# soedinglab/plass

Hardware: AMD Instinct MI355X
Metric: read-overlaps/s per assembly iteration (higher is better)
Workload: dtype u8/u64 (integer hash, byte compare; f32 ratios)

## Files before the change

### plass_amd/csrc/kmermatch.hip

```cpp
#include "common.hpp"
#include "device_utils.hpp"
#include "host_util.hpp"
#include "linepart.hpp"
#include "ref_rules.hpp"
#include "xxh64_u64.hpp"
#include <algorithm>
#include <memory>
#include <type_traits>
#include <cstdlib>
#include <climits>
#include <cstring>

namespace plasship {

#include "kmermatch_extract.hpp"
#include "kmermatch_group.hpp"
#include "kmermatch_repsort.hpp"
}
using namespace plasship;

namespace {

struct Timer {
    plasship_ctx *ctx; int slot;
// ... 72 lines not shown
    g.PL1 = pieceLinesFor(g.totalLines, g.nb1, numCU, 8);
    g.nP1 = (g.totalLines + g.PL1 - 1) / g.PL1;
    g.cap1 = std::max<uint64_t>(g.nP1 * ((uint64_t) g.PL1 + g.nb1), 1);
    if (g.nb2) {
        g.PL2 = 0xFFFFFFFFu; g.maxP2 = g.nb1; g.cap2 = g.cap1 + (uint64_t) g.nb1 * g.nb2;
    }
    return g;
}
static uint64_t repLevel1Cap(uint64_t nRec, uint64_t nSeg, uint32_t PL, uint32_t nb) {
    const uint64_t lines = (nRec + RPL - 1) / RPL + nSeg;
    return lines + (lines / PL + nSeg + 1) * (uint64_t) nb;
}

__global__ void arenaStartKernel(const uint32_t *__restrict__ lineBeg, uint32_t bpb, uint32_t gGrid, uint32_t nBuckets, uint64_t *__restrict__ arenaStart) {
    for (uint32_t j = blockIdx.x * blockDim.x + threadIdx.x; j < gGrid; j += gridDim.x * blockDim.x)
        arenaStart[j] = (uint64_t) lineBeg[std::min(j * bpb, nBuckets - 1)] * RPL;
}
__global__ void bigNeedKernel(const uint32_t *__restrict__ lineCnt, const uint32_t *__restrict__ unique, uint32_t nBuckets, uint64_t *__restrict__ need, uint32_t wordsPerEntry) {
    for (uint32_t b = blockIdx.x * blockDim.x + threadIdx.x; b < nBuckets; b += gridDim.x * blockDim.x) {
        const uint64_t c = (uint64_t) lineCnt[b] * RPL;
        uint64_t v = 0;
        if (unique[b] == AGG_NEEDS_SCRATCH) { uint64_t P = 1; while (P < c) P <<= 1; v = wordsPerEntry * P; }
        need[b] = v;
    }
}
__global__ void sumU32Kernel(const uint32_t *__restrict__ v, uint32_t n, unsigned long long *__restrict__ out) {
    unsigned long long s = 0;
    for (uint32_t i = blockIdx.x * blockDim.x + threadIdx.x; i < n; i += gridDim.x * blockDim.x) s += v[i];
    s = waveReduceSumU64(s);
    if (laneId() == 0 && s) atomicAdd(out, s);
}

template <class K> static int setDynLds(K k, size_t bytes) {
    PH_CHECK(hipFuncSetAttribute(reinterpret_cast<const void *>(k), hipFuncAttributeMaxDynamicSharedMemorySize, (int) bytes));
    return PLASSHIP_OK;
}
template <bool NUCL, bool LONG, int MODE, bool LIST, bool EXTRAS>
static int launchLinePart(plasship_ctx *ctx, const LinePartArgs &a, uint64_t nPiecesBound) {
    const size_t lds = linePartLdsBytes(a.nb, sizeof(Rec<LONG>), EXTRAS);
    const bool big = lds > 72 * 1024;
    const unsigned grid = (unsigned) std::max<uint64_t>(1, std::min<uint64_t>(nPiecesBound, (uint64_t) ctx->numCU * (big ? 1u : 2u)));
    if (big) {
        constexpr bool HASH = MODE == KEY_HASH;
        auto k = linePartKernel<NUCL, LONG, MODE, LIST, EXTRAS, 1024, (HASH && !LIST) ? 2 : 4, true, HASH, HASH>;
        const int rc = setDynLds(k, lds); if (rc) return rc;
        hipLaunchKernelGGL(k, dim3(grid), dim3(1024), lds, ctx->stream, a);
    } else {
        auto k = linePartKernel<NUCL, LONG, MODE, LIST, EXTRAS, 512, 4, true>;
        const int rc = setDynLds(k, lds); if (rc) return rc;
        hipLaunchKernelGGL(k, dim3(grid), dim3(512), lds, ctx->stream, a);
    }
    return PLASSHIP_OK;
}

static bool lineListDebugOn() { return getenv("PLASSHIP_DEBUG_LINELIST") != nullptr; }

static int buildLineLists(plasship_ctx *ctx, const char *who, const uint32_t *dTags, uint64_t capLines, uint32_t nb, uint32_t *dCount, uint32_t *dStart, uint32_t *dCursor, uint32_t *dList) {
    hipStream_t st = ctx->stream;
    PH_CHECK(hipMemsetAsync(dCount, 0, (size_t) nb * 4, st));
    const unsigned g = (unsigned) std::max<uint64_t>(1, std::min<uint64_t>((capLines + 4095) / 4096, (uint64_t) ctx->numCU * 8));
    const size_t lds = listRunsLdsBytes(LR_CHUNK, false);
    const unsigned gs = (unsigned) std::max<uint64_t>(1, std::min<uint64_t>((capLines + LR_CHUNK - 1) / LR_CHUNK, (uint64_t) ctx->numCU));
    auto k = tagScatterRunsKernel<LR_BLOCK, LR_CHUNK>;
    const int rc = setDynLds(k, lds); if (rc) return rc;
    hipLaunchKernelGGL(tagHistKernel, dim3(g), dim3(256), 0, st, dTags, capLines, nb, dCount);
    hipLaunchKernelGGL(tagScanKernel, dim3(1), dim3(1024), 0, st, (const uint32_t *) dCount, nb, dStart, dCursor);
    hipLaunchKernelGGL(k, dim3(gs), dim3(LR_BLOCK), lds, st, dTags, capLines, nb, dCursor, dList);
    if (lineListDebugOn()) {
        std::vector<uint32_t> s((size_t) nb + 1);
        PH_COPY_SYNC(st, s.data(), dStart, s.size() * 4, hipMemcpyDeviceToHost);
        uint32_t mx = 0; for (uint32_t b = 0; b < nb; b++) mx = std::max(mx, s[b + 1] - s[b]);
        fprintf(stderr, "lineList %s level 1 buckets %u lines %llu listed %u chunk %d chunks %llu regions 0 maxBucket %u\n", who, nb, (unsigned long long) capLines, s[nb], LR_CHUNK,
                (unsigned long long) ((capLines + LR_CHUNK - 1) / LR_CHUNK), mx);
    }
    return PLASSHIP_OK;
}
static int buildRegionLists(plasship_ctx *ctx, const char *who, const uint32_t *dTags, const uint32_t *dNPieces, const uint64_t *dRegBeg, const uint64_t *dRegEnd, uint32_t nRegions, uint32_t nb2, uint32_t *dList, uint32_t *dFineBeg, uint32_t *dFineCnt) {
    hipStream_t st = ctx->stream;
    const size_t lds = listRunsLdsBytes(LR2_CHUNK, true);
    auto k = tagSortRegionRunsKernel<LR2_BLOCK, LR2_CHUNK>;
    const int rc = setDynLds(k, lds); if (rc) return rc;
    hipLaunchKernelGGL(k, dim3(std::max<uint32_t>(1, std::min<uint32_t>(nRegions, (uint32_t) ctx->numCU))), dim3(LR2_BLOCK), lds, st, dTags, dRegBeg, dRegEnd, nRegions, nb2, dList, dFineBeg, dFineCnt);
    if (lineListDebugOn()) {
        std::vector<uint64_t> rb(nRegions), re(nRegions); std::vector<uint32_t> fc((size_t) nRegions * nb2);
        PH_COPY_SYNC(st, rb.data(), dRegBeg, rb.size() * 8, hipMemcpyDeviceToHost); PH_COPY_SYNC(st, re.data(), dRegEnd, re.size() * 8, hipMemcpyDeviceToHost);
        PH_COPY_SYNC(st, fc.data(), dFineCnt, fc.size() * 4, hipMemcpyDeviceToHost);
        uint32_t nPieces = 0; PH_COPY_SYNC(st, &nPieces, dNPieces, 4, hipMemcpyDeviceToHost);
        uint64_t lines = 0, listed = 0, chunks = 0, maxRegion = 0; uint32_t mx = 0, emptyRegions = 0;
        for (uint32_t g = 0; g < nRegions; g++) {
            const uint64_t len = re[g] - rb[g]; lines += len; chunks += (len + LR2_CHUNK - 1) / LR2_CHUNK;
            uint64_t in = 0; for (uint32_t f = 0; f < nb2; f++) { const uint32_t c = fc[(size_t) g * nb2 + f]; in += c; mx = std::max(mx, c); }
            listed += in; maxRegion = std::max(maxRegion, in); emptyRegions += in == 0;
        }
        fprintf(stderr, "lineList %s level 2 buckets %u lines %llu listed %llu chunk %d chunks %llu regions %u maxBucket %u emptyRegions %u maxRegion %llu pieces %u\n", who, nb2, (unsigned long long) lines,
                (unsigned long long) listed, LR2_CHUNK, (unsigned long long) chunks, nRegions, mx, emptyRegions, (unsigned long long) maxRegion, nPieces);
    }
    return PLASSHIP_OK;
}

static bool shardOwnerFiltered(int W) { const int m = tuneInt("SHARD_EXTRACT", 0); return m == 2 || (m != 1 && W <= 4); }

constexpr int KM_RETRY_EARLY_OVERFLOW_CHECK = -1000;
struct LinesOut { void *triples = nullptr; uint64_t nTriples = 0, Nk = 0, Nm = 0; std::vector<int64_t> stalePos; uint32_t staleT = 0; float msSort1 = 0, msGroup = 0, msSort2 = 0, msPart = 0; int nPart = 1;
                  uint64_t exchangedRecordBytes = 0, exchangedTripleBytes = 0; };

constexpr uint64_t HALO_SLACK = 1u << 16;
// ... 738 lines not shown
        bool fast = k == KF;
        uint64_t pwH = 1; for (int i = 0; i < HF; i++) pwH *= sa.base;
        if (pwH * 2 >= (1ull << 32)) fast = false;
        sa.topLo = (uint32_t) (pwH / sa.base); sa.topHi = (uint32_t) ea.powers[KF - HF - 1]; sa.baseH = (uint32_t) pwH;
        const dim3 shortGrid(std::min<uint32_t>((nMine + 63) / 64, (uint32_t) ctx->numCU * (nMine > 20000000u ? 288u : 18u)));
        const bool allWork = (int64_t) db->maxEntryLen - 2 - k + 1 <= (int64_t) par->kmers_per_seq - 1;
        const size_t padLds = (size_t) (allWork ? 16 : 8) << 10;
        const bool staged = !LONG && allWork;
        if (fast && sa.base < (1u << 8) && sa.topLo < (1u << 24) && sa.topHi < (1u << 24) && staged) {
            if constexpr (!LONG) hipLaunchKernelGGL((extractShortFastKernel<LONG, KF, true, true>), shortGrid, dim3(64), 0, st, sa);
        }
        else if (fast && sa.base < (1u << 8) && sa.topLo < (1u << 24) && sa.topHi < (1u << 24)) hipLaunchKernelGGL((extractShortFastKernel<LONG, KF, true>), shortGrid, dim3(64), padLds, st, sa);
        else if (fast) hipLaunchKernelGGL((extractShortFastKernel<LONG, KF, false>), shortGrid, dim3(64), 0, st, sa);
        else hipLaunchKernelGGL((extractShortKernel<LONG>), shortGrid, dim3(64), 0, st, sa);
        ea.waveList = dWaveList.as<uint32_t>(); ea.waveCount = dWaveCount.as<uint32_t>();
        if (cacheReuse) {
            CachedArgs ca; memset(&ca, 0, sizeof(ca));
            ca.s = ea.s; ca.slotOff = ea.slotOff; ca.arr = ea.arr; ca.map = ea.map; ca.lines = kc.lines.as<unsigned char>();
            ca.list = dCachedList.as<uint32_t>(); ca.count = dCachedCount.as<uint32_t>(); ca.k = k; ca.xCode = ea.xCode;
            ca.base = (uint32_t) ea.powers[1]; ca.base7 = (uint32_t) ea.powers[7]; ca.slotBias = slotBias; ca.seed = ea.seed; ca.kstats = dKStats.as<unsigned long long>();
            hipLaunchKernelGGL(extractCachedKernel, dim3(std::min<uint32_t>(nMine, (uint32_t) ctx->numCU * 32u)), dim3(64), 0, st, ca);
        }
    }
    else if (nMine) {
        hipLaunchKernelGGL(classifyWindowsKernel, dim3(std::min<uint32_t>((nMine + 2047) / 2048, (uint32_t) ctx->numCU * 8)), dim3(256), 0, st, (const uint32_t *) db->d_len.as<uint32_t>(), sLo, sHi, (uint32_t) k,
                           TIER0_WINDOWS, 64u * 16u, dWaveList.as<uint32_t>(), dWaveCount.as<uint32_t>(), dLongList.as<uint32_t>(), dLongCount.as<uint32_t>(), dOvIds.as<uint32_t>(), dOvCnt.as<uint32_t>(),
                           posReuse ? (const uint32_t *) db->d_origin.as<uint32_t>() : (const uint32_t *) nullptr, dCachedList.as<uint32_t>(), dCachedCount.as<uint32_t>());
        ea.waveList = dWaveList.as<uint32_t>(); ea.waveCount = dWaveCount.as<uint32_t>();
        if constexpr (NUCL) {
            if (posReuse) {
                CachedPosArgs<LONG> ca; memset(&ca, 0, sizeof(ca));
                ca.s = ea.s; ca.slotOff = ea.slotOff; ca.arr = ea.arr; ca.map = ea.map; ca.posOld = pc.pos.p; ca.slotOffOld = pc.slotOff.as<uint64_t>();
                ca.idHashOld = pc.idHash.as<unsigned long long>(); ca.origin = db->d_origin.as<uint32_t>(); ca.posNew = dPosNew.p; ca.idHashNew = dIdHashNew.as<unsigned long long>();
                ca.list = dCachedList.as<uint32_t>(); ca.count = dCachedCount.as<uint32_t>(); ca.k = k; ca.seed = ea.seed; ca.kstats = dKStats.as<unsigned long long>();
                hipLaunchKernelGGL((extractCachedPosKernel<LONG>), dim3(std::min<uint32_t>(nMine, (uint32_t) ctx->numCU * 32u)), dim3(64), 0, st, ca);
            }
        }
    }
    PH_CHECK(hipEventRecord(ctx->ev[3], st));
    PH_CHECK(hipEventRecord(ctx->ev[4], st));
    const int waveBlocksPerCU = nMine > 5000000u ? 192 : 32;
    DevBuf dOv2Ids, dOv2Cnt;
    DevBuf *lastIds = &dOvIds, *lastCnt = &dOvCnt;
    if (nMine) {
        if (dOv2Ids.alloc(((size_t) N + 1) * 4) != hipSuccess || dOv2Cnt.alloc(4) != hipSuccess) { setError("kmermatch: out of device memory"); return PLASSHIP_ERR_DEVICE; }
        PH_CHECK(hipMemsetAsync(dOv2Cnt.p, 0, 4, st));
        const uint32_t wide = std::min<uint32_t>(nMine, (uint32_t) ctx->numCU * (uint32_t) waveBlocksPerCU);
        ExtractArgs e0 = ea;
        DevBuf dRowLists, dRowCounts, dRowFall, dRowFallCnt;
        const bool rowTier = !NUCL && !LONG && fastIndex && k <= 14 && par->kmers_per_seq >= 1 && par->kmers_per_seq <= (int) KMC_POS + 1 &&
                             par->kmers_per_seq_scale == 0.0f && (tuneInt("ROWTIER", nMine > 4000000u ? 1 : 2) & 1) == 1;
        if (rowTier) {
            const uint32_t rs = N + 1;
            if (dRowLists.alloc((size_t) 4 * rs * 4) != hipSuccess || dRowCounts.alloc(16) != hipSuccess || dRowFall.alloc((size_t) rs * 4) != hipSuccess || dRowFallCnt.alloc(4) != hipSuccess) {
                setError("kmermatch: out of device memory"); return PLASSHIP_ERR_DEVICE;
            }
            PH_CHECK(hipMemsetAsync(dRowCounts.p, 0, 16, st));
            PH_CHECK(hipMemsetAsync(dRowFallCnt.p, 0, 4, st));
            hipLaunchKernelGGL(binWaveListKernel, dim3(std::min<uint32_t>((nMine + 2047) / 2048, (uint32_t) ctx->numCU * 8)), dim3(256), 0, st, (const uint32_t *) dWaveList.as<uint32_t>(), (const uint32_t *) dWaveCount.as<uint32_t>(),
                               (const uint32_t *) db->d_len.as<uint32_t>(), (uint32_t) k, 96u, 128u, 192u, dRowLists.as<uint32_t>(), rs, dRowCounts.as<uint32_t>());
            RowArgs ra; memset(&ra, 0, sizeof(ra));
            ra.s = ea.s; ra.slotOff = ea.slotOff; ra.arr = ea.arr; ra.map = ea.map; ra.fallList = dRowFall.as<uint32_t>(); ra.fallCount = dRowFallCnt.as<uint32_t>();
            ra.k = k; ra.xCode = ea.xCode; ra.kps = ea.kps; ra.ignoreMulti = ea.ignoreMulti; ra.seed = ea.seed; ra.base = (uint32_t) ea.powers[1]; ra.base7 = (uint32_t) ea.powers[7];
            ra.slotBias = slotBias; ra.kstats = dKStats.as<unsigned long long>();
            const dim3 rowGrid(std::min<uint32_t>((nMine + 3) / 4, (uint32_t) ctx->numCU * 32u));
            for (int b = 0; b < 4; b++) {
                ra.list = dRowLists.as<uint32_t>() + (size_t) b * rs; ra.count = dRowCounts.as<uint32_t>() + b;
                if (b == 0) hipLaunchKernelGGL((extractRowKernel<6>), rowGrid, dim3(64), 0, st, ra);
                else if (b == 1) hipLaunchKernelGGL((extractRowKernel<8>), rowGrid, dim3(64), 0, st, ra);
                else if (b == 2) hipLaunchKernelGGL((extractRowKernel<12>), rowGrid, dim3(64), 0, st, ra);
                else hipLaunchKernelGGL((extractRowKernel<16>), rowGrid, dim3(64), 0, st, ra);
            }
            e0.waveList = dRowFall.as<uint32_t>(); e0.waveCount = dRowFallCnt.as<uint32_t>();
        }
        hipLaunchKernelGGL((extractKernel<NUCL, LONG, CAP, false, 4, 256>), dim3(wide), dim3(64), 0, st, e0);
        ExtractArgs e1 = ea; e1.waveList = dLongList.as<uint32_t>(); e1.waveCount = dLongCount.as<uint32_t>();
        hipLaunchKernelGGL((extractKernel<NUCL, LONG, CAP, false, 16, 992>), dim3(wide), dim3(64), 0, st, e1);
        ExtractArgs e2 = ea; e2.waveList = dOvIds.as<uint32_t>(); e2.waveCount = dOvCnt.as<uint32_t>();
        e2.overflowIds = dOv2Ids.as<uint32_t>(); e2.overflowCount = dOv2Cnt.as<uint32_t>();
        constexpr int CAP48 = NUCL ? 512 : 128;
        if constexpr (NUCL) hipLaunchKernelGGL((extractKernel<NUCL, LONG, CAP48, false, 48, 992, 2>), dim3(std::min<uint32_t>(nMine, (uint32_t) ctx->numCU * 8u)), dim3(64), 0, st, e2);
        else hipLaunchKernelGGL((extractKernel<NUCL, LONG, CAP2, false, 48, 992>), dim3(std::min<uint32_t>(nMine, (uint32_t) ctx->numCU * 16u)), dim3(64), 0, st, e2);
        PH_CHECK(hipMemsetAsync(dOvCnt.p, 0, 4, st));
        ExtractArgs e3 = ea; e3.waveList = dOv2Ids.as<uint32_t>(); e3.waveCount = dOv2Cnt.as<uint32_t>();
        e3.overflowIds = dOvIds.as<uint32_t>(); e3.overflowCount = dOvCnt.as<uint32_t>();
        hipLaunchKernelGGL((extractKernel<NUCL, LONG, CAP2, false, 0, 8160>), dim3(std::min<uint32_t>(nMine, (uint32_t) ctx->numCU * (NUCL ? 2u : 5u))), dim3(64), 0, st, e3);
    }
    DevBuf &dLastIds = *lastIds, &dLastCnt = *lastCnt;
    PH_CHECK(hipEventRecord(ctx->ev[5], st));
    uint32_t nOv = 0;
    const bool overflowPossible = overflowCheckEarly || cm != nullptr || NUCL || db->maxEntryLen > 8160u || par->kmers_per_seq > 120 || par->kmers_per_seq_scale != 0.0f;
    if (nMine && overflowPossible) {
        PH_CHECK(hipMemcpyAsync(&nOv, dLastCnt.p, 4, hipMemcpyDeviceToHost, st));
        PH_CHECK(plasship::streamSync(st));
    } else if (nMine) hipLaunchKernelGGL((fillOverflowSlotsKernel<LONG>), dim3(64), dim3(64), 0, st, (const uint32_t *) dLastIds.as<uint32_t>(), (const uint32_t *) dLastCnt.as<uint32_t>(),
                                         (const uint64_t *) dSlotOff.as<uint64_t>(), slotBias, dA.p);
    PH_CHECK(hipGetLastError());
    if (nOv) {
        std::vector<uint32_t> ids(nOv), lens(nOv);
        DevBuf dLens, dSOff, dSCap, dScratch;
        if (dLens.alloc((size_t) nOv * 4) != hipSuccess) { setError("kmermatch: out of device memory"); return PLASSHIP_ERR_DEVICE; }
        hipLaunchKernelGGL(gatherU32Kernel, dim3(gridFor(nOv, 256, 1024)), dim3(256), 0, st, db->d_len.as<uint32_t>(), dLastIds.as<uint32_t>(), nOv, dLens.as<uint32_t>());
        PH_CHECK(hipMemcpyAsync(lens.data(), dLens.p, (size_t) nOv * 4, hipMemcpyDeviceToHost, st));
        PH_CHECK(plasship::streamSync(st));
        std::vector<uint64_t> soff(nOv); std::vector<uint32_t> scap(nOv); uint64_t tot = 0;
        for (uint32_t i = 0; i < nOv; i++) { uint32_t c = 64; while (c < lens[i] + 1) c <<= 1; scap[i] = c; soff[i] = tot; tot += c; }
        if (dSOff.alloc((size_t) nOv * 8) != hipSuccess || dSCap.alloc((size_t) nOv * 4) != hipSuccess || dScratch.alloc(tot * sizeof(Cand)) != hipSuccess) {
            setError("kmermatch: out of device memory for the long-sequence scratch"); return PLASSHIP_ERR_DEVICE;
        }
        PH_CHECK(hipMemcpyAsync(dSOff.p, soff.data(), (size_t) nOv * 8, hipMemcpyHostToDevice, st));
        PH_CHECK(hipMemcpyAsync(dSCap.p, scap.data(), (size_t) nOv * 4, hipMemcpyHostToDevice, st));
        ExtractArgs fa = ea; fa.idList = dLastIds.as<uint32_t>(); fa.nIds = nOv; fa.scratch = dScratch.as<Cand>(); fa.scratchOff = dSOff.as<uint64_t>(); fa.scratchCap = dSCap.as<uint32_t>();
        hipLaunchKernelGGL((extractKernel<NUCL, LONG, 1, true>), dim3(std::min<uint32_t>(nOv, (uint32_t) ctx->numCU * 8)), dim3(64), 0, st, fa);
        PH_CHECK(plasship::streamSync(st));
        PH_CHECK(hipGetLastError());
    }
    PH_TRACE(st, "kmermatch: extraction");
    traceBadIds<LONG>(ctx, "kmermatch: extracted slots", dA.p, total, N);

    {
        int keyBitsL = 0;
        if (NUCL) keyBitsL = 2 * k; else { long double v = 1; for (int i = 0; i < k; i++) v *= (long double) (alph - 1); while (keyBitsL < 63 && (long double) (1ULL << keyBitsL) < v) keyBitsL++; }
        LinesOut lo;
        int rcL = kmermatchLines<NUCL, LONG>(ctx, db, par, geo, total, dA, dB, dSlotOff, dKStats, ea, keyBitsL, lo, (nMine && !overflowPossible) ? dLastCnt.as<uint32_t>() : nullptr, filtered);
        if (rcL) return rcL;
        std::unique_ptr<plasship_cands> holderL; uint64_t NcL = 0; float msReduceL = 0;
        rcL = reduceToCandidates<NUCL, LONG>(ctx, db, lo.triples, lo.nTriples, lo.stalePos, lo.staleT, holderL, NcL, msReduceL, true);
        if (rcL) return rcL;
        {
            auto ms = [&](int a, int b) { float v = 0; (void) hipEventElapsedTime(&v, ctx->ev[a], ctx->ev[b]); return v; };
// ... 51 lines not shown
```

### plass_amd/csrc/kmermatch_extract.hpp

```cpp
#pragma once

__device__ __forceinline__ uint64_t revComplementDev(uint64_t kmer, int k) {
    uint64_t x = kmer ^ 0xAAAAAAAAAAAAAAAAULL;
    x = ((x >> 2) & 0x3333333333333333ULL) | ((x & 0x3333333333333333ULL) << 2);
    x = ((x >> 4) & 0x0F0F0F0F0F0F0F0FULL) | ((x & 0x0F0F0F0F0F0F0F0FULL) << 4);
    x = __builtin_bswap64(x);
    return x >> (64 - 2 * k);
}

__global__ void boundsKernel(const uint32_t *__restrict__ len, uint32_t n, int k, int kps, float scale, uint32_t *__restrict__ bound) {
    for (uint32_t i = blockIdx.x * blockDim.x + threadIdx.x; i < n; i += gridDim.x * blockDim.x) {
        const int L = (int) len[i];
        const int adj = max(1, L - k + 2);
        bound[i] = (uint32_t) min(adj, (int) ((float) (size_t) kps + (scale * (float) L)));
    }
}

struct Cand { uint64_t kmer; uint32_t pos; uint32_t score; };
constexpr uint32_t KMC_LINE = 128, KMC_POS = 59, KMC_FLAGS = 63, KMC_CLEAN = 1;

#define FALLBACK_NOSTATS(a) ((a).kstats == nullptr)
struct ExtractArgs {
    SeqView s;
    const uint64_t *slotOff;
// ... 915 lines not shown
        m.idh = *reinterpret_cast<const unsigned long long *>(ln);
        return m;
    };
    Meta nxt; nxt.id = 0; nxt.L = 0; nxt.pos = 0xFFFFu; nxt.off = 0; nxt.slot = 0; nxt.slot1 = 0; nxt.idh = 0;
    uint32_t id2 = 0;
    if (blockIdx.x < nWork) nxt = loadMeta(a.list[blockIdx.x]);
    if (blockIdx.x + gridDim.x < nWork) id2 = a.list[blockIdx.x + gridDim.x];
    for (uint32_t w = blockIdx.x; w < nWork; w += gridDim.x) {
        const Meta cur = nxt;
        if (w + gridDim.x < nWork) nxt = loadMeta(id2);
        if (w + 2 * gridDim.x < nWork) id2 = a.list[w + 2 * gridDim.x];
        const char *base = a.s.data + cur.off;
        const uint32_t bound = (uint32_t) (cur.slot1 - cur.slot);
        const bool have = cur.pos != 0xFFFFu;
        const uint32_t n = (uint32_t) __popcll(__ballot(have));
        if (have) {
            uint64_t r0, r1; __builtin_memcpy(&r0, base + cur.pos, 8); __builtin_memcpy(&r1, base + cur.pos + 8, 8);
            uint64_t w0 = 0, w1 = 0;
#pragma unroll
            for (int b = 0; b < 8; b++) { w0 |= (uint64_t) sMap[(r0 >> (8 * b)) & 0xFF] << (8 * b); w1 |= (uint64_t) sMap[(r1 >> (8 * b)) & 0xFF] << (8 * b); }
            uint64_t kmer; (void) kmerIndexCore(w0, w1, a.k, (unsigned) a.xCode, a.base, a.base7, kmer);
            R r; r.kmer = kmer; r.id = cur.id; r.len = (uint16_t) cur.L; r.pos = (int16_t) cur.pos;
            arr[cur.slot + 1 + (uint32_t) lane] = r;
        }
        if (lane == 63) { R r; r.kmer = xxh64U64(cur.idh, a.seed); r.id = cur.id; r.len = (uint16_t) cur.L; r.pos = 0; arr[cur.slot] = r; }
        for (uint32_t i = 1 + n + (uint32_t) lane; i < bound; i += 64) { R r; memset(&r, 0xFF, sizeof(R)); arr[cur.slot + i] = r; }
        stRes += cur.L; stRec += 1 + n;
    }
    if (lane == 0 && a.kstats) { atomicAdd(&a.kstats[2], stRes); atomicAdd(&a.kstats[3], stRec); }
}

struct RowArgs {
    SeqView s; const uint64_t *slotOff; void *arr; const unsigned char *map;
    const uint32_t *list, *count;
    uint32_t *fallList, *fallCount;
    int k, xCode, kps, ignoreMulti; uint64_t seed; uint32_t base, base7; uint64_t slotBias;
    unsigned long long *kstats;
};
constexpr uint64_t rowPowU64(uint64_t b, unsigned e) { uint64_t r = 1; while (e) { if (e & 1u) r *= b; b *= b; e >>= 1; } return r; }
constexpr uint64_t rowInv31() { uint64_t x = 31; for (int i = 0; i < 6; i++) x *= 2ull - 31ull * x; return x; }
static_assert(rowInv31() * 31ull == 1ull, "inverse of 31 modulo 2^64");
__device__ __forceinline__ uint32_t rowExclusiveScan16(uint32_t v) {
    uint32_t x = v;
    x += (uint32_t) __builtin_amdgcn_update_dpp(0, (int) x, 0x111, 0xF, 0xF, true);
    x += (uint32_t) __builtin_amdgcn_update_dpp(0, (int) x, 0x112, 0xF, 0xF, true);
    x += (uint32_t) __builtin_amdgcn_update_dpp(0, (int) x, 0x114, 0xF, 0xF, true);
    x += (uint32_t) __builtin_amdgcn_update_dpp(0, (int) x, 0x118, 0xF, 0xF, true);
    return x - v;
}
__device__ __forceinline__ unsigned long long rowSum16U64(unsigned long long v) {
    v += dppMov64<0xB1>(v); v += dppMov64<0x4E>(v); v += dppMov64<0x141>(v); v += dppMov64<0x140>(v);
    return v;
}
__global__ __launch_bounds__(256) void binWaveListKernel(const uint32_t *__restrict__ list, const uint32_t *__restrict__ count, const uint32_t *__restrict__ len, uint32_t k,
                                                         uint32_t w0, uint32_t w1, uint32_t w2, uint32_t *__restrict__ out, uint32_t outStride, uint32_t *__restrict__ outCount) {
    __shared__ uint32_t sCnt[4], sBase[4];
    const uint32_t n = *count;
    constexpr int PER = 8;
    for (uint64_t b0 = (uint64_t) blockIdx.x * (256 * PER); b0 < n; b0 += (uint64_t) gridDim.x * (256 * PER)) {
        if (threadIdx.x < 4) sCnt[threadIdx.x] = 0;
        __syncthreads();
        int cls[PER]; uint32_t rank[PER], ids[PER];
#pragma unroll
        for (int j = 0; j < PER; j++) {
            const uint64_t i = b0 + (uint64_t) j * 256 + threadIdx.x;
            cls[j] = -1; rank[j] = 0; ids[j] = 0;
            if (i < n) {
                ids[j] = list[i];
                const uint32_t L = len[ids[j]], nw = L >= k ? L - k + 1 : 0u;
                cls[j] = nw <= w0 ? 0 : (nw <= w1 ? 1 : (nw <= w2 ? 2 : 3));
                rank[j] = atomicAdd(&sCnt[cls[j]], 1u);
            }
        }
        __syncthreads();
        if (threadIdx.x < 4) sBase[threadIdx.x] = sCnt[threadIdx.x] ? atomicAdd(&outCount[threadIdx.x], sCnt[threadIdx.x]) : 0u;
        __syncthreads();
#pragma unroll
        for (int j = 0; j < PER; j++) if (cls[j] >= 0) out[(size_t) cls[j] * outStride + sBase[cls[j]] + rank[j]] = ids[j];
        __syncthreads();
    }
}

template <int REGS>
__global__ __launch_bounds__(64) __attribute__((amdgpu_waves_per_eu(4))) void extractRowKernel(RowArgs a) {
    constexpr uint32_t MAXWIN = 16u * REGS, MAXL = MAXWIN + 13u;
    constexpr uint32_t ROWB = (MAXL + 31u + 15u) & ~15u;
    constexpr bool TWO = MAXL > 256u;
    constexpr uint32_t NPOW = MAXL + 17u;
    __shared__ unsigned char sMap[256];
    __shared__ __attribute__((aligned(16))) unsigned char sCode[4][ROWB];
    __shared__ unsigned long long sPow[NPOW];
    __shared__ unsigned short sSel[4][64];
    __shared__ __attribute__((aligned(16))) uint32_t sSet[4][128];
    typedef Rec<false> R;
    R *arr = reinterpret_cast<R *>(a.arr);
    const int lane = threadIdx.x, row = lane >> 4, sub = lane & 15;
    const int k = a.k;
    if (blockIdx.x * 4u >= *a.count) return;
    for (int i = lane; i < 256; i += 64) sMap[i] = a.map[i];
    {
        constexpr uint64_t inv31 = rowInv31(), c0 = rowPowU64(inv31, 15), p64 = rowPowU64(31ull, 64);
        uint64_t m = c0;
#pragma unroll
        for (int b = 0; b < 6; b++) if ((lane >> b) & 1) m *= rowPowU64(31ull, 1u << b);
        for (uint32_t x = lane; x < NPOW; x += 64) { sPow[x] = m; m *= p64; }
    }
    __syncthreads();
    const uint32_t nWork = *a.count;
    const uint32_t stride = gridDim.x * 4u;
    const uint32_t xC = (uint32_t) a.xCode;
    const uint32_t considerRaw = (uint32_t) (a.kps - 1);
    unsigned long long stRes = 0, stRec = 0;
    struct Meta { uint32_t id, L; uint64_t off, slot, slot1; };
    auto loadMeta = [&](uint32_t w) {
        Meta m; m.id = 0xFFFFFFFFu; m.L = 0; m.off = 0; m.slot = 0; m.slot1 = 0;
        if (w < nWork) { m.id = a.list[w]; m.L = a.s.len[m.id]; m.off = a.s.off[m.id]; m.slot = a.slotOff[m.id] - a.slotBias; m.slot1 = a.slotOff[m.id + 1] - a.slotBias; }
        return m;
    };
    auto loadRaw = [&](const Meta &m, uint32_t at) { uint4 v = make_uint4(0, 0, 0, 0); if (at < m.L) __builtin_memcpy(&v, a.s.data + m.off + at, 16); return v; };
    uint32_t w = blockIdx.x * 4u + (uint32_t) row;
    auto loadId = [&](uint32_t ww) { return ww < nWork ? a.list[ww] : 0xFFFFFFFFu; };
    auto metaOf = [&](uint32_t id) {
        Meta m; m.id = id; m.L = 0; m.off = 0; m.slot = 0; m.slot1 = 0;
        if (id != 0xFFFFFFFFu) { m.L = a.s.len[id]; m.off = a.s.off[id]; m.slot = a.slotOff[id] - a.slotBias; m.slot1 = a.slotOff[id + 1] - a.slotBias; }
        return m;
    };
    Meta mNext = loadMeta(w); uint32_t id2 = loadId(w + stride);
    uint4 rawN0 = loadRaw(mNext, (uint32_t) sub * 16u);
    for (uint32_t w0 = blockIdx.x * 4u; w0 < nWork; w0 += stride, w += stride) {
        const Meta cur = mNext; const uint4 raw0 = rawN0;
        uint4 raw1 = make_uint4(0, 0, 0, 0);
        if (TWO) raw1 = loadRaw(cur, 256u + (uint32_t) sub * 16u);
        mNext = metaOf(id2);
        rawN0 = loadRaw(mNext, (uint32_t) sub * 16u);
        id2 = loadId(w + 2u * stride);
        const bool active = cur.id != 0xFFFFFFFFu;
        const uint32_t L = cur.L, id = cur.id;
        const uint32_t nWin = (L >= (uint32_t) k) ? L - (uint32_t) k + 1u : 0u;
        const bool tooLong = active && nWin > MAXWIN;
        const uint32_t nWinU = (uint32_t) __builtin_amdgcn_readfirstlane((int) waveMaxU32((active && !tooLong) ? nWin : 0u));
        unsigned long long hAcc = 0;
        auto stageChunk = [&](const uint4 &raw, uint32_t c) {
            const uint32_t r[4] = {raw.x, raw.y, raw.z, raw.w};
            uint32_t cw[4];
#pragma unroll
            for (int d = 0; d < 4; d++)
                cw[d] = (uint32_t) sMap[r[d] & 0xFFu] | ((uint32_t) sMap[(r[d] >> 8) & 0xFFu] << 8) | ((uint32_t) sMap[(r[d] >> 16) & 0xFFu] << 16) | ((uint32_t) sMap[r[d] >> 24] << 24);
            if (16u * c < ROWB) *reinterpret_cast<uint4 *>(&sCode[row][16u * c]) = make_uint4(cw[0], cw[1], cw[2], cw[3]);
            const int m = (int) L - (int) (16u * c);
            if (m > 0 && !tooLong) {
                uint32_t q[4];
#pragma unroll
                for (int d = 0; d < 4; d++) {
                    const int nb = m - 4 * d;
                    const uint32_t z = nb >= 4 ? cw[d] : (nb <= 0 ? 0u : (cw[d] & ((1u << (8 * nb)) - 1u)));
                    q[d] = __umul24(__umul24(__umul24(z & 0xFFu, 31u) + ((z >> 8) & 0xFFu), 31u) + ((z >> 16) & 0xFFu), 31u) + (z >> 24);
                }
                constexpr unsigned long long K4 = 923521ull;
                const unsigned long long H = (((unsigned long long) q[0] * K4 + q[1]) * K4 + q[2]) * K4 + q[3];
                hAcc += H * sPow[(uint32_t) ((int) L - 16 * (int) (c + 1) + 15)];
            }
        };
        stageChunk(raw0, (uint32_t) sub);
        if (TWO) stageChunk(raw1, 16u + (uint32_t) sub);
        if (active && !tooLong) for (uint32_t i = (uint32_t) sub; i < 31u; i += 16u) sCode[row][L + i] = (unsigned char) xC;
        for (uint32_t i = (uint32_t) sub * 4u; i < 128u; i += 64u) *reinterpret_cast<uint4 *>(&sSet[row][i]) = make_uint4(0, 0, 0, 0);
        __syncthreads();
        const unsigned long long seqHash = rowSum16U64(hAcc);
        uint32_t sc[REGS];
        uint32_t nLane = 0;
#pragma unroll
        for (int j = 0; j < REGS; j++) {
            sc[j] = 0xFFFFFFFFu;
            if ((uint32_t) j * 16u < nWinU) {
                const uint32_t p = (uint32_t) j * 16u + (uint32_t) sub;
                uint64_t kmer;
                const bool v = kmerIndexFastAligned(sCode[row], p, k, xC, a.base, a.base7, kmer);
                const uint32_t h = xxh64Score16(kmer, a.seed);
                const bool use = v && p < nWin && !tooLong;
                sc[j] = use ? h : 0xFFFFFFFFu; nLane += use ? 1u : 0u;
            }
            __builtin_amdgcn_sched_barrier(0);
        }
        const uint32_t n = (uint32_t) rowSum16((int) nLane);
        const uint32_t considered = min(considerRaw, n);
        uint32_t t = 0;
#pragma unroll 1
        for (int bit = 15; bit >= 0; bit--) {
            const uint32_t tr = t | (1u << bit);
            uint32_t c = 0;
#pragma unroll
            for (int j = 0; j < REGS; j++) if ((uint32_t) j * 16u < nWinU) c += (sc[j] < tr) ? 1u : 0u;
            if ((uint32_t) rowSum16((int) c) < considered) t = tr;
        }
        if (n <= considered) t = 0xFFFFu;
        uint32_t selMask = 0;
#pragma unroll
        for (int j = 0; j < REGS; j++) if ((uint32_t) j * 16u < nWinU) selMask |= (sc[j] <= t) ? (1u << j) : 0u;
        const uint32_t cLane = (uint32_t) __popc(selMask);
        const uint32_t C = (uint32_t) rowSum16((int) cLane);
        bool ok = active && !tooLong && C == considered;
        {
            uint32_t at = rowExclusiveScan16(cLane);
            if (ok) {
#pragma unroll
                for (int j = 0; j < REGS; j++) if ((selMask >> j) & 1u) { sSel[row][at] = (unsigned short) ((uint32_t) j * 16u + (uint32_t) sub); at++; }
            }
        }
        __syncthreads();
        const uint64_t slot = cur.slot;
        const uint32_t bound = (uint32_t) (cur.slot1 - cur.slot);
        bool rep = false;
#pragma unroll
        for (int i = 0; i < 4; i++) {
            const uint32_t r = (uint32_t) sub + 16u * (uint32_t) i;
            if (ok && r < C) {
                const uint32_t p = sSel[row][r];
                uint64_t kmer; (void) kmerIndexFastAligned(sCode[row], p, k, xC, a.base, a.base7, kmer);
                if (a.ignoreMulti) {
                    const uint64_t hx = kmer * 0x9E3779B97F4A7C15ULL;
                    const uint32_t tag = (uint32_t) (hx >> 32) | 1u;
                    uint32_t sl = (uint32_t) (hx >> 20) & 127u;
                    for (;;) {
                        const uint32_t prev = atomicCAS(&sSet[row][sl], 0u, tag);
                        if (prev == 0u) break;
                        if (prev == tag) { rep = true; break; }
                        sl = (sl + 1u) & 127u;
                    }
                }
                R rec; rec.kmer = kmer; rec.id = id; rec.len = (uint16_t) L; rec.pos = (int16_t) p;
                arr[slot + 1 + r] = rec;
            }
            __builtin_amdgcn_sched_barrier(0);
        }
        if (rowSum16(rep ? 1 : 0) != 0) ok = false;
        if (ok) {
            if (sub == 15) { R rec; rec.kmer = xxh64U64(seqHash, a.seed); rec.id = id; rec.len = (uint16_t) L; rec.pos = 0; arr[slot] = rec; }
            for (uint32_t i = 1u + C + (uint32_t) sub; i < bound; i += 16u) { R rec; memset(&rec, 0xFF, sizeof(R)); arr[slot + i] = rec; }
            unsigned char *cl = reinterpret_cast<unsigned char *>(a.kstats[4]);
            if (cl) {
                unsigned short *ln = reinterpret_cast<unsigned short *>(cl + (size_t) id * KMC_LINE);
#pragma unroll
                for (int i = 0; i < 4; i++) { const uint32_t r = (uint32_t) sub + 16u * (uint32_t) i; if (r < KMC_POS) ln[4 + r] = (r < C) ? sSel[row][r] : (unsigned short) 0xFFFFu; }
                if (sub == 0) *reinterpret_cast<unsigned long long *>(ln) = seqHash;
                if (sub == 15) ln[KMC_FLAGS] = (unsigned short) KMC_CLEAN;
            }
            if (sub == 0) { stRes += L; stRec += 1 + C; }
        }
        {
            const bool fall = active && !ok && sub == 0;
            const unsigned long long fm = __ballot(fall);
            if (fm) {
                uint32_t basePos = 0;
                if (lane == 0) basePos = atomicAdd(a.fallCount, (uint32_t) __popcll(fm));
                basePos = __shfl(basePos, 0, 64);
                if (fall) a.fallList[basePos + (uint32_t) __popcll(fm & ((1ULL << lane) - 1ULL))] = id;
            }
        }
        __syncthreads();
    }
    stRes = waveReduceSumU64(stRes); stRec = waveReduceSumU64(stRec);
    if (lane == 0 && a.kstats) { atomicAdd(&a.kstats[2], stRes); atomicAdd(&a.kstats[3], stRec); }
}

template <bool LONG>
struct CachedPosArgs {
    SeqView s; const uint64_t *slotOff; void *arr; const unsigned char *map;
    const void *posOld; const uint64_t *slotOffOld; const unsigned long long *idHashOld; const uint32_t *origin;
    void *posNew; unsigned long long *idHashNew;
    const uint32_t *list, *count; int k; uint64_t seed; unsigned long long *kstats;
};
template <bool LONG>
__global__ __launch_bounds__(64) void extractCachedPosKernel(CachedPosArgs<LONG> a) {
    __shared__ unsigned char sMap[256];
    typedef Rec<LONG> R;
    typedef typename std::conditional<LONG, uint32_t, unsigned short>::type PosT;
    R *arr = reinterpret_cast<R *>(a.arr);
    const PosT *posOld = reinterpret_cast<const PosT *>(a.posOld);
    PosT *posNew = reinterpret_cast<PosT *>(a.posNew);
    const int lane = threadIdx.x;
    for (int i = lane; i < 256; i += 64) sMap[i] = a.map[i];
    __syncthreads();
    const int k = a.k;
    const uint32_t nWork = *a.count;
    unsigned long long stRes = 0, stRec = 0;
    struct Meta { uint32_t id, L, cnt; uint64_t off, slot, slot1, so; unsigned long long idh; };
    auto loadMeta = [&](uint32_t id) {
        Meta m; m.id = id; m.L = a.s.len[id]; m.off = a.s.off[id]; m.slot = a.slotOff[id]; m.slot1 = a.slotOff[id + 1];
        const uint32_t src = a.origin[id];
        m.so = a.slotOffOld[src]; m.idh = a.idHashOld[src]; m.cnt = (uint32_t) posOld[m.so];
        return m;
    };
    Meta nxt; nxt.id = 0; nxt.L = 0; nxt.cnt = 0; nxt.off = 0; nxt.slot = 0; nxt.slot1 = 0; nxt.so = 0; nxt.idh = 0;
    if (blockIdx.x < nWork) nxt = loadMeta(a.list[blockIdx.x]);
    for (uint32_t w = blockIdx.x; w < nWork; w += gridDim.x) {
        const Meta cur = nxt;
        if (w + gridDim.x < nWork) nxt = loadMeta(a.list[w + gridDim.x]);
        const char *base = a.s.data + cur.off;
// ... 55 lines not shown
```

Before: 758.9 million.

## Extend row-tier extraction to long sequences with 32- and 64-lane groups

Generalizes extractRowKernel to process one sequence per 16, 32 or 64 lanes, using permlane16/32 swaps to join row reductions and scans, and splits the power table for the 64-lane case. Long-list sequences (windows up to 1024) are now binned by length and routed through these row kernels, with only the fallbacks sent to the generic extractKernel<16,992>. The aim is to replace the slower generic long-sequence extraction with the register-resident selection path. The cost is extra binning and kernel launches, more device buffers, and a debug-only host readback.

```diff
diff --git a/plass_amd/csrc/kmermatch.hip b/plass_amd/csrc/kmermatch.hip
--- a/plass_amd/csrc/kmermatch.hip
+++ b/plass_amd/csrc/kmermatch.hip
@@ -148,6 +148,9 @@
     }
     return PLASSHIP_OK;
 }
+
+static bool rowTierDebugOn() { return getenv("PLASSHIP_DEBUG_ROWTIER") != nullptr; }
+static constexpr uint32_t ROW_WIDE_BINS[3] = {320u, 384u, 512u};
 
 static bool lineListDebugOn() { return getenv("PLASSHIP_DEBUG_LINELIST") != nullptr; }
 
@@ -992,10 +995,10 @@
                              par->kmers_per_seq_scale == 0.0f && (tuneInt("ROWTIER", nMine > 4000000u ? 1 : 2) & 1) == 1;
         if (rowTier) {
             const uint32_t rs = N + 1;
-            if (dRowLists.alloc((size_t) 4 * rs * 4) != hipSuccess || dRowCounts.alloc(16) != hipSuccess || dRowFall.alloc((size_t) rs * 4) != hipSuccess || dRowFallCnt.alloc(4) != hipSuccess) {
+            if (dRowLists.alloc((size_t) 4 * rs * 4) != hipSuccess || dRowCounts.alloc(48) != hipSuccess || dRowFall.alloc((size_t) rs * 4) != hipSuccess || dRowFallCnt.alloc(4) != hipSuccess) {
                 setError("kmermatch: out of device memory"); return PLASSHIP_ERR_DEVICE;
             }
-            PH_CHECK(hipMemsetAsync(dRowCounts.p, 0, 16, st));
+            PH_CHECK(hipMemsetAsync(dRowCounts.p, 0, 48, st));
             PH_CHECK(hipMemsetAsync(dRowFallCnt.p, 0, 4, st));
             hipLaunchKernelGGL(binWaveListKernel, dim3(std::min<uint32_t>((nMine + 2047) / 2048, (uint32_t) ctx->numCU * 8)), dim3(256), 0, st, (const uint32_t *) dWaveList.as<uint32_t>(), (const uint32_t *) dWaveCount.as<uint32_t>(),
                                (const uint32_t *) db->d_len.as<uint32_t>(), (uint32_t) k, 96u, 128u, 192u, dRowLists.as<uint32_t>(), rs, dRowCounts.as<uint32_t>());
@@ -1015,7 +1018,42 @@
         }
         hipLaunchKernelGGL((extractKernel<NUCL, LONG, CAP, false, 4, 256>), dim3(wide), dim3(64), 0, st, e0);
         ExtractArgs e1 = ea; e1.waveList = dLongList.as<uint32_t>(); e1.waveCount = dLongCount.as<uint32_t>();
+        DevBuf dWideLists, dWideFall;
+        if (rowTier) {
+            const uint32_t rs = N + 1;
+            if (dWideLists.alloc((size_t) 4 * rs * 4) != hipSuccess || dWideFall.alloc((size_t) rs * 4) != hipSuccess) { setError("kmermatch: out of device memory"); return PLASSHIP_ERR_DEVICE; }
+            uint32_t *wideCounts = dRowCounts.as<uint32_t>() + 4, *wideFallCnt = dRowCounts.as<uint32_t>() + 8;
+            hipLaunchKernelGGL(binWaveListKernel, dim3(std::min<uint32_t>((nMine + 2047) / 2048, (uint32_t) ctx->numCU * 8)), dim3(256), 0, st, (const uint32_t *) dLongList.as<uint32_t>(), (const uint32_t *) dLongCount.as<uint32_t>(),
+                               (const uint32_t *) db->d_len.as<uint32_t>(), (uint32_t) k, ROW_WIDE_BINS[0], ROW_WIDE_BINS[1], ROW_WIDE_BINS[2], dWideLists.as<uint32_t>(), rs, wideCounts);
+            RowArgs ra; memset(&ra, 0, sizeof(ra));
+            ra.s = ea.s; ra.slotOff = ea.slotOff; ra.arr = ea.arr; ra.map = ea.map; ra.fallList = dWideFall.as<uint32_t>(); ra.fallCount = wideFallCnt;
+            ra.k = k; ra.xCode = ea.xCode; ra.kps = ea.kps; ra.ignoreMulti = ea.ignoreMulti; ra.seed = ea.seed; ra.base = (uint32_t) ea.powers[1]; ra.base7 = (uint32_t) ea.powers[7];
+            ra.slotBias = slotBias; ra.kstats = dKStats.as<unsigned long long>();
+            const dim3 pairGrid(std::min<uint32_t>((nMine + 1) / 2, (uint32_t) ctx->numCU * 32u)), oneGrid(std::min<uint32_t>(nMine, (uint32_t) ctx->numCU * 32u));
+            for (int b = 0; b < 4; b++) {
+                ra.list = dWideLists.as<uint32_t>() + (size_t) b * rs; ra.count = wideCounts + b;
+                if (b == 0) hipLaunchKernelGGL((extractRowKernel<10, 32>), pairGrid, dim3(64), 0, st, ra);
+                else if (b == 1) hipLaunchKernelGGL((extractRowKernel<12, 32>), pairGrid, dim3(64), 0, st, ra);
+                else if (b == 2) hipLaunchKernelGGL((extractRowKernel<16, 32>), pairGrid, dim3(64), 0, st, ra);
+                else hipLaunchKernelGGL((extractRowKernel<16, 64>), oneGrid, dim3(64), 0, st, ra);
+            }
+            e1.waveList = dWideFall.as<uint32_t>(); e1.waveCount = wideFallCnt;
+        }
         hipLaunchKernelGGL((extractKernel<NUCL, LONG, CAP, false, 16, 992>), dim3(wide), dim3(64), 0, st, e1);
+        if (rowTier && rowTierDebugOn()) {
+            uint32_t c[12], fell16 = 0;
+            PH_COPY_SYNC(st, c, dRowCounts.p, sizeof(c), hipMemcpyDeviceToHost);
+            PH_COPY_SYNC(st, &fell16, dRowFallCnt.p, 4, hipMemcpyDeviceToHost);
+            uint32_t nLong = 0;
+            PH_COPY_SYNC(st, &nLong, dLongCount.p, 4, hipMemcpyDeviceToHost);
+            std::vector<uint32_t> ids(nLong), lens(N);
+            if (nLong) PH_COPY_SYNC(st, ids.data(), dLongList.p, (size_t) nLong * 4, hipMemcpyDeviceToHost);
+            if (N) PH_COPY_SYNC(st, lens.data(), db->d_len.p, (size_t) N * 4, hipMemcpyDeviceToHost);
+            uint32_t hist[24] = {0};
+            for (uint32_t id : ids) { const uint32_t nw = lens[id] - (uint32_t) k + 1; if (nw > 256u && nw <= 1024u) hist[(nw - 257u) / 32u]++; }
+            std::string h; for (int i = 0; i < 24; i++) h += (i ? "," : "") + std::to_string(hist[i]);
+            fprintf(stderr, "rowTier rows16 %u %u %u %u fell %u rows32 %u %u %u rows64 %u fell %u of %u hist %s\n", c[0], c[1], c[2], c[3], fell16, c[4], c[5], c[6], c[7], c[8], nLong, h.c_str());
+        }
         ExtractArgs e2 = ea; e2.waveList = dOvIds.as<uint32_t>(); e2.waveCount = dOvCnt.as<uint32_t>();
         e2.overflowIds = dOv2Ids.as<uint32_t>(); e2.overflowCount = dOv2Cnt.as<uint32_t>();
         constexpr int CAP48 = NUCL ? 512 : 128;
diff --git a/plass_amd/csrc/kmermatch_extract.hpp b/plass_amd/csrc/kmermatch_extract.hpp
--- a/plass_amd/csrc/kmermatch_extract.hpp
+++ b/plass_amd/csrc/kmermatch_extract.hpp
@@ -991,6 +991,37 @@
     v += dppMov64<0xB1>(v); v += dppMov64<0x4E>(v); v += dppMov64<0x141>(v); v += dppMov64<0x140>(v);
     return v;
 }
+template <int LANES> struct RowGroup {
+    static_assert(LANES == 16 || LANES == 32 || LANES == 64, "a group is one, two or four rows of 16 lanes");
+    static __device__ __forceinline__ void joinRows(uint32_t t, uint32_t &lo, uint32_t &all) {
+        lo = 0; all = t;
+        if constexpr (LANES >= 32) {
+            const auto r = __builtin_amdgcn_permlane16_swap(t, t, false, false);
+            lo = (threadIdx.x & 16u) ? r[0] : 0u; all = r[0] + r[1];
+        }
+        if constexpr (LANES == 64) {
+            const auto q = __builtin_amdgcn_permlane32_swap(all, all, false, false);
+            lo += (threadIdx.x & 32u) ? q[0] : 0u; all = q[0] + q[1];
+        }
+    }
+    static __device__ __forceinline__ uint32_t sum(uint32_t v) { uint32_t lo, all; joinRows((uint32_t) rowSum16((int) v), lo, all); return all; }
+    static __device__ __forceinline__ uint32_t exclusiveScan(uint32_t v) {
+        uint32_t lo, all; joinRows((uint32_t) rowSum16((int) v), lo, all);
+        return rowExclusiveScan16(v) + lo;
+    }
+    static __device__ __forceinline__ unsigned long long sumU64(unsigned long long v) {
+        v = rowSum16U64(v);
+        if constexpr (LANES >= 32) {
+            const auto l = __builtin_amdgcn_permlane16_swap((uint32_t) v, (uint32_t) v, false, false), h = __builtin_amdgcn_permlane16_swap((uint32_t) (v >> 32), (uint32_t) (v >> 32), false, false);
+            v = (((unsigned long long) h[0] << 32) | l[0]) + (((unsigned long long) h[1] << 32) | l[1]);
+        }
+        if constexpr (LANES == 64) {
+            const auto l = __builtin_amdgcn_permlane32_swap((uint32_t) v, (uint32_t) v, false, false), h = __builtin_amdgcn_permlane32_swap((uint32_t) (v >> 32), (uint32_t) (v >> 32), false, false);
+            v = (((unsigned long long) h[0] << 32) | l[0]) + (((unsigned long long) h[1] << 32) | l[1]);
+        }
+        return v;
+    }
+};
 __global__ __launch_bounds__(256) void binWaveListKernel(const uint32_t *__restrict__ list, const uint32_t *__restrict__ count, const uint32_t *__restrict__ len, uint32_t k,
                                                          uint32_t w0, uint32_t w1, uint32_t w2, uint32_t *__restrict__ out, uint32_t outStride, uint32_t *__restrict__ outCount) {
     __shared__ uint32_t sCnt[4], sBase[4];
@@ -1020,33 +1051,47 @@
     }
 }
 
-template <int REGS>
+template <int REGS, int LANES = 16>
 __global__ __launch_bounds__(64) __attribute__((amdgpu_waves_per_eu(4))) void extractRowKernel(RowArgs a) {
-    constexpr uint32_t MAXWIN = 16u * REGS, MAXL = MAXWIN + 13u;
+    static_assert(LANES == 16 || LANES == 32 || LANES == 64, "a group is one, two or four rows of 16 lanes");
+    constexpr int GROUPS = 64 / LANES;
+    constexpr uint32_t MAXWIN = (uint32_t) LANES * REGS, MAXL = MAXWIN + 13u;
     constexpr uint32_t ROWB = (MAXL + 31u + 15u) & ~15u;
-    constexpr bool TWO = MAXL > 256u;
+    constexpr bool TWO = MAXL > 16u * LANES;
+    static_assert(MAXL <= 32u * LANES, "two chunks of 16 bytes per lane hold the longest sequence");
     constexpr uint32_t NPOW = MAXL + 17u;
     __shared__ unsigned char sMap[256];
-    __shared__ __attribute__((aligned(16))) unsigned char sCode[4][ROWB];
-    __shared__ unsigned long long sPow[NPOW];
-    __shared__ unsigned short sSel[4][64];
-    __shared__ __attribute__((aligned(16))) uint32_t sSet[4][128];
+    __shared__ __attribute__((aligned(16))) unsigned char sCode[GROUPS][ROWB];
+    constexpr bool SPLIT = LANES == 64;
+    constexpr uint32_t NHI = (NPOW + 15u) / 16u;
+    __shared__ unsigned long long sPow[SPLIT ? NHI + 16u : NPOW];
+    __shared__ unsigned short sSel[GROUPS][64];
+    __shared__ __attribute__((aligned(16))) uint32_t sSet[GROUPS][128];
     typedef Rec<false> R;
+    typedef RowGroup<LANES> G;
     R *arr = reinterpret_cast<R *>(a.arr);
-    const int lane = threadIdx.x, row = lane >> 4, sub = lane & 15;
+    const int lane = threadIdx.x, row = lane / LANES, sub = lane % LANES;
     const int k = a.k;
-    if (blockIdx.x * 4u >= *a.count) return;
+    if (blockIdx.x * (uint32_t) GROUPS >= *a.count) return;
     for (int i = lane; i < 256; i += 64) sMap[i] = a.map[i];
     {
         constexpr uint64_t inv31 = rowInv31(), c0 = rowPowU64(inv31, 15), p64 = rowPowU64(31ull, 64);
         uint64_t m = c0;
 #pragma unroll
-        for (int b = 0; b < 6; b++) if ((lane >> b) & 1) m *= rowPowU64(31ull, 1u << b);
-        for (uint32_t x = lane; x < NPOW; x += 64) { sPow[x] = m; m *= p64; }
+        for (int b = 0; b < 6; b++) if ((lane >> b) & 1) m *= rowPowU64(31ull, (SPLIT ? 16u : 1u) << b);
+        if constexpr (SPLIT) {
+            for (uint32_t x = lane; x < NHI; x += 64) { sPow[x] = m; m *= rowPowU64(31ull, 1024); }
+            uint64_t l = 1;
+#pragma unroll
+            for (int b = 0; b < 4; b++) if ((lane >> b) & 1) l *= rowPowU64(31ull, 1u << b);
+            if (lane < 16) sPow[NHI + (uint32_t) lane] = l;
+        } else {
+            for (uint32_t x = lane; x < NPOW; x += 64) { sPow[x] = m; m *= p64; }
+        }
     }
     __syncthreads();
     const uint32_t nWork = *a.count;
-    const uint32_t stride = gridDim.x * 4u;
+    const uint32_t stride = gridDim.x * (uint32_t) GROUPS;
     const uint32_t xC = (uint32_t) a.xCode;
     const uint32_t considerRaw = (uint32_t) (a.kps - 1);
     unsigned long long stRes = 0, stRec = 0;
@@ -1057,7 +1102,7 @@
         return m;
     };
     auto loadRaw = [&](const Meta &m, uint32_t at) { uint4 v = make_uint4(0, 0, 0, 0); if (at < m.L) __builtin_memcpy(&v, a.s.data + m.off + at, 16); return v; };
-    uint32_t w = blockIdx.x * 4u + (uint32_t) row;
+    uint32_t w = blockIdx.x * (uint32_t) GROUPS + (uint32_t) row;
     auto loadId = [&](uint32_t ww) { return ww < nWork ? a.list[ww] : 0xFFFFFFFFu; };
     auto metaOf = [&](uint32_t id) {
         Meta m; m.id = id; m.L = 0; m.off = 0; m.slot = 0; m.slot1 = 0;
@@ -1066,10 +1111,10 @@
     };
     Meta mNext = loadMeta(w); uint32_t id2 = loadId(w + stride);
     uint4 rawN0 = loadRaw(mNext, (uint32_t) sub * 16u);
-    for (uint32_t w0 = blockIdx.x * 4u; w0 < nWork; w0 += stride, w += stride) {
+    for (uint32_t w0 = blockIdx.x * (uint32_t) GROUPS; w0 < nWork; w0 += stride, w += stride) {
         const Meta cur = mNext; const uint4 raw0 = rawN0;
         uint4 raw1 = make_uint4(0, 0, 0, 0);
-        if (TWO) raw1 = loadRaw(cur, 256u + (uint32_t) sub * 16u);
+        if (TWO) raw1 = loadRaw(cur, 16u * LANES + (uint32_t) sub * 16u);
         mNext = metaOf(id2);
         rawN0 = loadRaw(mNext, (uint32_t) sub * 16u);
         id2 = loadId(w + 2u * stride);
@@ -1097,22 +1142,23 @@
                 }
                 constexpr unsigned long long K4 = 923521ull;
                 const unsigned long long H = (((unsigned long long) q[0] * K4 + q[1]) * K4 + q[2]) * K4 + q[3];
-                hAcc += H * sPow[(uint32_t) ((int) L - 16 * (int) (c + 1) + 15)];
+                const uint32_t e = (uint32_t) ((int) L - 16 * (int) (c + 1) + 15);
+                hAcc += H * (SPLIT ? sPow[e >> 4] * sPow[NHI + (e & 15u)] : sPow[e]);
             }
         };
         stageChunk(raw0, (uint32_t) sub);
-        if (TWO) stageChunk(raw1, 16u + (uint32_t) sub);
-        if (active && !tooLong) for (uint32_t i = (uint32_t) sub; i < 31u; i += 16u) sCode[row][L + i] = (unsigned char) xC;
-        for (uint32_t i = (uint32_t) sub * 4u; i < 128u; i += 64u) *reinterpret_cast<uint4 *>(&sSet[row][i]) = make_uint4(0, 0, 0, 0);
+        if (TWO) stageChunk(raw1, (uint32_t) LANES + (uint32_t) sub);
+        if (active && !tooLong) for (uint32_t i = (uint32_t) sub; i < 31u; i += (uint32_t) LANES) sCode[row][L + i] = (unsigned char) xC;
+        for (uint32_t i = (uint32_t) sub * 4u; i < 128u; i += 4u * LANES) *reinterpret_cast<uint4 *>(&sSet[row][i]) = make_uint4(0, 0, 0, 0);
         __syncthreads();
-        const unsigned long long seqHash = rowSum16U64(hAcc);
+        const unsigned long long seqHash = G::sumU64(hAcc);
         uint32_t sc[REGS];
         uint32_t nLane = 0;
 #pragma unroll
         for (int j = 0; j < REGS; j++) {
             sc[j] = 0xFFFFFFFFu;
-            if ((uint32_t) j * 16u < nWinU) {
-                const uint32_t p = (uint32_t) j * 16u + (uint32_t) sub;
+            if ((uint32_t) j * LANES < nWinU) {
+                const uint32_t p = (uint32_t) j * LANES + (uint32_t) sub;
                 uint64_t kmer;
                 const bool v = kmerIndexFastAligned(sCode[row], p, k, xC, a.base, a.base7, kmer);
                 const uint32_t h = xxh64Score16(kmer, a.seed);
@@ -1121,7 +1167,7 @@
             }
             __builtin_amdgcn_sched_barrier(0);
         }
-        const uint32_t n = (uint32_t) rowSum16((int) nLane);
+        const uint32_t n = G::sum(nLane);
         const uint32_t considered = min(considerRaw, n);
         uint32_t t = 0;
 #pragma unroll 1
@@ -1129,21 +1175,21 @@
             const uint32_t tr = t | (1u << bit);
             uint32_t c = 0;
 #pragma unroll
-            for (int j = 0; j < REGS; j++) if ((uint32_t) j * 16u < nWinU) c += (sc[j] < tr) ? 1u : 0u;
-            if ((uint32_t) rowSum16((int) c) < considered) t = tr;
+            for (int j = 0; j < REGS; j++) if ((uint32_t) j * LANES < nWinU) c += (sc[j] < tr) ? 1u : 0u;
+            if (G::sum(c) < considered) t = tr;
         }
         if (n <= considered) t = 0xFFFFu;
         uint32_t selMask = 0;
 #pragma unroll
-        for (int j = 0; j < REGS; j++) if ((uint32_t) j * 16u < nWinU) selMask |= (sc[j] <= t) ? (1u << j) : 0u;
+        for (int j = 0; j < REGS; j++) if ((uint32_t) j * LANES < nWinU) selMask |= (sc[j] <= t) ? (1u << j) : 0u;
         const uint32_t cLane = (uint32_t) __popc(selMask);
-        const uint32_t C = (uint32_t) rowSum16((int) cLane);
+        const uint32_t C = G::sum(cLane);
         bool ok = active && !tooLong && C == considered;
         {
-            uint32_t at = rowExclusiveScan16(cLane);
+            uint32_t at = G::exclusiveScan(cLane);
             if (ok) {
 #pragma unroll
-                for (int j = 0; j < REGS; j++) if ((selMask >> j) & 1u) { sSel[row][at] = (unsigned short) ((uint32_t) j * 16u + (uint32_t) sub); at++; }
+                for (int j = 0; j < REGS; j++) if ((selMask >> j) & 1u) { sSel[row][at] = (unsigned short) ((uint32_t) j * LANES + (uint32_t) sub); at++; }
             }
         }
         __syncthreads();
@@ -1151,8 +1197,8 @@
         const uint32_t bound = (uint32_t) (cur.slot1 - cur.slot);
         bool rep = false;
 #pragma unroll
-        for (int i = 0; i < 4; i++) {
-            const uint32_t r = (uint32_t) sub + 16u * (uint32_t) i;
+        for (int i = 0; i < GROUPS; i++) {
+            const uint32_t r = (uint32_t) sub + (uint32_t) LANES * (uint32_t) i;
             if (ok && r < C) {
                 const uint32_t p = sSel[row][r];
                 uint64_t kmer; (void) kmerIndexFastAligned(sCode[row], p, k, xC, a.base, a.base7, kmer);
@@ -1172,17 +1218,17 @@
             }
             __builtin_amdgcn_sched_barrier(0);
         }
-        if (rowSum16(rep ? 1 : 0) != 0) ok = false;
+        if (G::sum(rep ? 1u : 0u) != 0u) ok = false;
         if (ok) {
-            if (sub == 15) { R rec; rec.kmer = xxh64U64(seqHash, a.seed); rec.id = id; rec.len = (uint16_t) L; rec.pos = 0; arr[slot] = rec; }
-            for (uint32_t i = 1u + C + (uint32_t) sub; i < bound; i += 16u) { R rec; memset(&rec, 0xFF, sizeof(R)); arr[slot + i] = rec; }
+            if (sub == LANES - 1) { R rec; rec.kmer = xxh64U64(seqHash, a.seed); rec.id = id; rec.len = (uint16_t) L; rec.pos = 0; arr[slot] = rec; }
+            for (uint32_t i = 1u + C + (uint32_t) sub; i < bound; i += (uint32_t) LANES) { R rec; memset(&rec, 0xFF, sizeof(R)); arr[slot + i] = rec; }
             unsigned char *cl = reinterpret_cast<unsigned char *>(a.kstats[4]);
             if (cl) {
                 unsigned short *ln = reinterpret_cast<unsigned short *>(cl + (size_t) id * KMC_LINE);
 #pragma unroll
-                for (int i = 0; i < 4; i++) { const uint32_t r = (uint32_t) sub + 16u * (uint32_t) i; if (r < KMC_POS) ln[4 + r] = (r < C) ? sSel[row][r] : (unsigned short) 0xFFFFu; }
+                for (int i = 0; i < GROUPS; i++) { const uint32_t r = (uint32_t) sub + (uint32_t) LANES * (uint32_t) i; if (r < KMC_POS) ln[4 + r] = (r < C) ? sSel[row][r] : (unsigned short) 0xFFFFu; }
                 if (sub == 0) *reinterpret_cast<unsigned long long *>(ln) = seqHash;
-                if (sub == 15) ln[KMC_FLAGS] = (unsigned short) KMC_CLEAN;
+                if (sub == LANES - 1) ln[KMC_FLAGS] = (unsigned short) KMC_CLEAN;
             }
             if (sub == 0) { stRes += L; stRec += 1 + C; }
         }
```

Measured after the change: 770.3 million, median of 6. +1.5%, better.
